# microsoft/timewarp

Measured on AMD Instinct MI355X. Metric: MH-accepted samples/sec (whole node), alanine-dipeptide kernel_transformer_nvp, higher is better.
Workload: dtype f16x3 (split-fp16 operands, 3 MFMAs per fp32 product, fp32 accumulate)

## Files before the change

### timewarp_amd/csrc/tw_api.hip

```cpp
#include "tw_common.h"

namespace tw {
std::atomic<int> g_debug_flags{0};
const char* last_error();
int launch_prior_logp(const float* zc, const float* zv, const uint8_t* masked, int64_t n_cond, const float* prior,
                      const float* delta, float sign, float* out, int64_t n_rows, int V, hipStream_t s);
int launch_uncentre_add(const float* xc, const float* com, const float* resid, int64_t n_cond, float* y, int V,
                        int displacement, int64_t n_rows, hipStream_t s);
int launch_sub(const float* a, const float* b, float* o, int64_t total, hipStream_t s);
int launch_kinetic(const float* v, const float* masses, int random_velocs, float kbT, float* out, int64_t n, int V,
                   hipStream_t s);
int launch_mh_accept(const float* energy, const float* p_xy, const float* p_yx, const float* u, const float* yc,
                     const float* yv, float* xc, float* xv, float* out_exp, float* out_pacc, uint8_t* out_acc,
                     int32_t* result, int64_t S, int V, hipStream_t s, int64_t n_chains = 1);
int launch_chirality(const float* coords, const int32_t* centres, const float* ref, int n_centres, uint8_t* changed,
                     int64_t n_rows, int V, hipStream_t s);
int amber_energy(const tw_forcefield* ff, const float* coords, double* out, double* terms, int64_t n, hipStream_t s);
int amber_energy_forces(const tw_forcefield* ff, const float* coords, double* out_energy, double* out_forces, int64_t n, hipStream_t s);
int langevin_steps(const tw_forcefield* ff, const float* masses, float* coords, float* velocs, int n_steps, double dt,
                   double friction, double kbT, int scheme, unsigned long long seed, long long step0, double* out_energy,
                   int64_t n, hipStream_t s);
}

using namespace tw;
// ... 135 lines not shown
  if (rc) return rc;
  TW_REQUIRE(h1_supported(*desc, 22), "single-MFMA path unsupported for this config");
  TW_REQUIRE(raw && packed_h1, "NULL buffer");
  return h3_pack_weights(*desc, raw, (char*)packed_h1, (hipStream_t)stream, true);
}

int64_t tw_flow_workspace_bytes(const tw_flow_desc* desc, int64_t n_rows, int32_t n_atoms) {
  if (check_desc(desc) || n_rows < 0 || n_atoms <= 0) return -1;
  const int64_t rows = n_rows > 0 ? n_rows : 1;
  int64_t a = simple_workspace_bytes(*desc, rows, n_atoms);
  int64_t b = fused_supported(*desc, n_atoms) ? fused_workspace_bytes(*desc, rows, n_atoms) : 0;
  if (h3_supported(*desc, n_atoms)) {
    const int64_t c = h3_workspace_bytes(*desc, rows, n_atoms);
    if (c > b) b = c;
  }
  const int64_t extra = 6 * ((rows * n_atoms * 3 * 4 + 255) / 256 * 256) + 4 * ((rows * 4 + 255) / 256 * 256);
  return (a > b ? a : b) + extra;
}

int tw_flow_pass(const tw_flow_desc* desc, const float* raw, const float* packed, const int32_t* atom_types,
                 const float* x_coords, const float* x_velocs, const uint8_t* masked, int64_t n_cond, float* z_coords,
                 float* z_velocs, float* delta_logp, int64_t n_rows, int32_t n_atoms, int32_t reverse, int32_t path,
                 void* workspace, int64_t workspace_bytes, void* stream) {
  int rc = check_desc(desc);
  if (rc) return rc;
  TW_REQUIRE(n_rows >= 0 && n_atoms > 0 && n_cond > 0, "bad sizes");
  TW_REQUIRE(n_rows % n_cond == 0, "n_rows (%lld) must be a multiple of n_cond (%lld)", (long long)n_rows,
             (long long)n_cond);
  if (n_rows == 0) return TW_OK;
  TW_REQUIRE(raw && atom_types && x_coords && x_velocs && masked && z_coords && z_velocs && delta_logp && workspace,
             "NULL pointer argument");
  int p;
  if ((rc = resolve_path(*desc, n_atoms, path, packed, &p))) return rc;
  FlowArgs a{desc, raw, packed, atom_types, x_coords, x_velocs, masked, n_cond, z_coords, z_velocs,
             delta_logp, n_rows, n_atoms, reverse, workspace, workspace_bytes, (hipStream_t)stream};
  if (p == TW_PATH_FUSED_H3 || p == TW_PATH_FUSED_H1) {
    a.h1 = p == TW_PATH_FUSED_H1 ? 1 : 0;
    return flow_pass_h3(a);
  }
  a.simple_h3 = p == TW_PATH_SIMPLE_H3 ? 1 : 0;
  return p == TW_PATH_FUSED ? flow_pass_fused(a) : flow_pass_simple(a);
}

static char* carve(char*& p, int64_t bytes) {
  char* r = p;
  p += (bytes + 255) / 256 * 256;
  return r;
}

int tw_flow_log_likelihood(const tw_flow_desc* desc, const float* raw, const float* packed, const int32_t* atom_types,
                           const float* x_coords, const float* x_velocs, const float* y_coords, const float* y_velocs,
                           const uint8_t* masked, float* out_logp, int64_t n_rows, int32_t n_atoms, int32_t path,
                           void* workspace, int64_t workspace_bytes, void* stream) {
  int rc = check_desc(desc);
  if (rc) return rc;
  TW_REQUIRE(n_rows >= 0 && n_atoms > 0, "bad sizes");
  if (n_rows == 0) return TW_OK;
  TW_REQUIRE(raw && atom_types && x_coords && x_velocs && y_coords && y_velocs && masked && out_logp && workspace,
             "NULL pointer argument");
  hipStream_t s = (hipStream_t)stream;
  const int64_t el = n_rows * n_atoms * 3;
  char* p = (char*)workspace;
  float* xc = (float*)carve(p, el * 4);
  float* zc = (float*)carve(p, el * 4);
  float* zv = (float*)carve(p, el * 4);
// ... 300 lines not shown
```

### timewarp_amd/csrc/tw_common.h

```cpp
#pragma once
#include <hip/hip_runtime.h>
#include <stdint.h>
#include <stdio.h>
#include <string.h>

#include <atomic>
#include <vector>

#include "../../include/timewarp_hip.h"

namespace tw {

void set_error(const char* fmt, ...);

#define TW_HIP_CHECK(expr)                                                              \
  do {                                                                                  \
    hipError_t _e = (expr);                                                             \
    if (_e != hipSuccess) {                                                             \
      tw::set_error("%s failed: %s (%s:%d)", #expr, hipGetErrorString(_e), __FILE__, __LINE__); \
      return TW_ERR_HIP;                                                                \
    }                                                                                   \
  } while (0)

#define TW_LAUNCH_CHECK() TW_HIP_CHECK(hipGetLastError())
// ... 72 lines not shown
struct PackedLayout {
  int64_t tiles_per_net;
  int64_t side_per_net;
  int64_t net_stride;
  int64_t total;
};
PackedLayout packed_layout(const tw_flow_desc& d);

struct FusedGeom {
  int nt;
  int mpw;
  int tile_mask;
};
bool fused_geom(int n_atoms, FusedGeom* g);
bool fused_geom_nt(int n_atoms, int nt, FusedGeom* g);

int launch_scores(const float* x, const uint8_t* masked, const float* ls, int H, int64_t B, int V,
                  int normalise, int use_mm, float* out, hipStream_t s, const float* coeffs = nullptr, int order = 0,
                  int force_zero = 0, _Float16* s_hi = nullptr, _Float16* s_lo = nullptr);
bool scores_split_direct(int V);
int launch_centre(const float* x, const uint8_t* masked, float* xc, float* com, int64_t n, int V,
                  hipStream_t s);

struct FlowArgs {
  const tw_flow_desc* desc;
  const float* raw;
  const float* packed;
  const int32_t* atom_types;
  const float* x_coords;
  const float* x_velocs;
  const uint8_t* masked;
  int64_t n_cond;
  float* z_coords;
  float* z_velocs;
  float* delta_logp;
  int64_t n_rows;
  int n_atoms;
  int reverse;
  void* ws;
  int64_t ws_bytes;
  hipStream_t stream;
  int h1 = 0;
  int simple_h3 = 0;
};
__device__ __forceinline__ float tw_cdist_mm(float qx, float qy, float qz, float mx, float my, float mz) {
#pragma clang fp contract(off)
  const float qn = (qx * qx + qy * qy) + qz * qz;
  const float mn = (mx * mx + my * my) + mz * mz;
  float acc = (-2.f * qx) * mx;
  acc = __builtin_fmaf(-2.f * qy, my, acc);
  acc = __builtin_fmaf(-2.f * qz, mz, acc);
  acc = acc + qn;
  acc = acc + mn;
  return sqrtf(fmaxf(acc, 0.f));
}

__device__ __forceinline__ float basis_value(float sc, const float* __restrict__ coeff, int order, float coeff_mean) {
  if (order <= 0) return expf(-(sc * sc));
  {
#pragma clang fp contract(off)
  const float x = sc * sc;
  const float rf = (x - 1.0f) / (x + 1.0f);
  const float rf2 = 2.0f * rf;
  float rprev = 1.0f, rcur = rf;
  float acc = (coeff[0] - coeff_mean) * rprev;
  if (order >= 2) acc = __builtin_fmaf(coeff[1] - coeff_mean, rcur, acc);
// ... 30 lines not shown
bool equivariant_desc_ok(const tw_flow_desc& d);
void equivariant_raw_layout(const tw_flow_desc& d, RawLayout* L);
int64_t equivariant_workspace_bytes(const tw_flow_desc& d, int64_t n_rows, int n_atoms);
int flow_pass_equivariant(const FlowArgs& a);
int debug_module_equivariant(const FlowArgs& a, int c, int net, const float* z_other, float* dump);
int flow_pass_fused(const FlowArgs& a);
int64_t simple_workspace_bytes(const tw_flow_desc& d, int64_t n_rows, int n_atoms);
int64_t fused_workspace_bytes(const tw_flow_desc& d, int64_t n_rows, int n_atoms);
int launch_coupling(const float* s_raw, const float* t, const uint8_t* masked, int64_t n_cond,
                    float* z_out, float* delta_logp, int64_t n_rows, int V, int reverse, hipStream_t s,
                    const float* z_in = nullptr, int* flag = nullptr);
int* nonfinite_flag_device_ptr();
inline int* flow_range_flag(const tw_flow_desc& d) { return d.range_flag ? d.range_flag : nonfinite_flag_device_ptr(); }

struct PrevCoupling {
  const float* s_raw;
  const float* t;
  const float* z_in;
  float* z_out;
  float* delta_logp;
  int* nonfinite;
  int reverse;
};
enum PackFormat { PACK_F32, PACK_PAIR, PACK_HI };
enum PackKind { PACK_TILES, PACK_FOLD, PACK_COPY, PACK_SCALAR };
struct PackGroup {
  const float* src;
  const float* wo;
  int64_t n;
};
struct PackOp {
  int kind, fmt, group;
  const float* src;
  const float* wo;
  int ld, rows_valid, cols_valid;
  int H, h;
  int row0, col0, n_ot, n_ks;
  int64_t n, n_pad;
  void* dst;
};
struct PackPlan {
  std::vector<PackGroup> groups;
  std::vector<PackOp> ops;
  int add_group(PackGroup g) { groups.push_back(g); return (int)groups.size() - 1; }
  int matrix_scale(const float* src, int64_t n) { return add_group({src, nullptr, n}); }
  int fold_scale(const float* wv, const float* wo, int H) { return add_group({wv, wo, H}); }
// ... 62 lines not shown
```

### timewarp_amd/csrc/tw_mh_step.hip

```cpp
#include "tw_common.h"

extern "C" int tw_flow_pass(const tw_flow_desc* desc, const float* raw, const float* packed, const int32_t* atom_types,
                            const float* x_coords, const float* x_velocs, const uint8_t* masked, int64_t n_cond,
                            float* z_coords, float* z_velocs, float* delta_logp, int64_t n_rows, int32_t n_atoms,
                            int32_t reverse, int32_t path, void* workspace, int64_t workspace_bytes, void* stream);
extern "C" int64_t tw_flow_workspace_bytes(const tw_flow_desc* desc, int64_t n_rows, int32_t n_atoms);

namespace tw {
int amber_energy(const tw_forcefield* ff, const float* coords, double* out, double* terms, int64_t n, hipStream_t s);

namespace {

__device__ __forceinline__ float wsum(float v) {
#pragma unroll
  for (int o = 32; o > 0; o >>= 1) v += __shfl_xor(v, o);
  return v;
}

__device__ __forceinline__ float row_prior(const float* zc, const float* zv, const uint8_t* mk, const float* prior, int V) {
  const float sc = expf(prior[0]), sv = expf(prior[1]);
  const float var_c = sc * sc, var_v = sv * sv;
  const float lsc = logf(sc), lsv = logf(sv);
  const float half_log_2pi = 0.91893853320467274178f;
  float ac = 0.f, av = 0.f;
  for (int i = threadIdx.x; i < 3 * V; i += 64) {
    const float keep = mk[i / 3] ? 0.f : 1.f;
    const float a = zc[i], b = zv[i];
    ac += keep * (-(a * a) / (2.f * var_c) - lsc - half_log_2pi);
// ... 37 lines not shown
  if (n < S) {
    for (int a = threadIdx.x; a < V; a += 64) {
      types_rep[n * V + a] = types[a];
      masked_rep[n * V + a] = masked[a];
    }
    const float p = row_prior(zc + n * 3 * V, zv + n * 3 * V, masked, prior, V);
    if (threadIdx.x == 0) {
      prior0[n] = p;
      delta[n] = 0.f;
    }
    return;
  }
  float com[3];
  row_com(x_coords, masked, V, com);
  for (int i = threadIdx.x; i < 3 * V; i += 64) {
    xc[i] = x_coords[i] - com[i % 3];
    zc[S * 3 * V + i] = x_coords[i];
  }
  if (threadIdx.x < 3) com_out[threadIdx.x] = com[threadIdx.x];
  const float ek = row_kinetic(x_velocs, masses, random_velocs, kbT, V);
  if (threadIdx.x == 0) ekin_x[0] = ek;
}

__global__ void mh_finish_kernel(float* __restrict__ zc , const float* __restrict__ yv,
                                 const float* __restrict__ x_coords, const float* __restrict__ x_velocs,
                                 const float* __restrict__ xc, const float* __restrict__ com,
                                 const uint8_t* __restrict__ masked, const float* __restrict__ masses,
                                 const float* __restrict__ prior0, float* __restrict__ delta, float* __restrict__ p_xy,
                                 float* __restrict__ ekin_y, uint8_t* __restrict__ chir, const int32_t* __restrict__ centres,
                                 const float* __restrict__ ref_signs, int n_centres, float* __restrict__ t_c,
                                 float* __restrict__ t_v, float* __restrict__ c_v, float* __restrict__ c_c,
                                 int displacement, int random_velocs, float kbT, int V) {
  extern __shared__ float ys[];
  const int64_t n = blockIdx.x;
  const float sgn = random_velocs ? 1.f : -1.f;
  float* zrow = zc + n * 3 * V;
  for (int i = threadIdx.x; i < 3 * V; i += 64) {
    const float base = xc[i] + com[i % 3];
    const float y = displacement ? base + zrow[i] : zrow[i];
    zrow[i] = y;
    ys[i] = y;
    t_c[n * 3 * V + i] = displacement ? x_coords[i] - y : x_coords[i];
    t_v[n * 3 * V + i] = sgn * x_velocs[i];
    c_v[n * 3 * V + i] = sgn * yv[n * 3 * V + i];
  }
  __syncthreads();
  float cy[3];
  row_com(ys, masked, V, cy);
  for (int i = threadIdx.x; i < 3 * V; i += 64) c_c[n * 3 * V + i] = ys[i] - cy[i % 3];
  const float ek = row_kinetic(yv + n * 3 * V, masses, random_velocs, kbT, V);
  if (threadIdx.x == 0) {
    p_xy[n] = prior0[n] + delta[n];
    delta[n] = 0.f;
    ekin_y[n] = ek;
    bool ch = false;
    for (int c = 0; c < n_centres; ++c) {
      const int i0 = centres[4 * c], i1 = centres[4 * c + 1], i2 = centres[4 * c + 2], i3 = centres[4 * c + 3];
      float a[3], b[3], d[3];
      for (int k = 0; k < 3; ++k) {
        a[k] = ys[3 * i1 + k] - ys[3 * i0 + k];
        b[k] = ys[3 * i2 + k] - ys[3 * i0 + k];
        d[k] = ys[3 * i3 + k] - ys[3 * i0 + k];
      }
      const float cx = b[1] * d[2] - b[2] * d[1];
      const float cyy = b[2] * d[0] - b[0] * d[2];
      const float cz = b[0] * d[1] - b[1] * d[0];
      const float dot = a[0] * cx + a[1] * cyy + a[2] * cz;
      const float s = (dot > 0.f) ? 1.f : ((dot < 0.f) ? -1.f : 0.f);
      if (s != ref_signs[c]) ch = true;
    }
    chir[n] = ch ? 1 : 0;
  }
}

__global__ void mh_pyx_kernel(const float* __restrict__ zc, const float* __restrict__ zv, const uint8_t* __restrict__ masked,
                              const float* __restrict__ prior, const float* __restrict__ delta, float* __restrict__ p_yx, int V) {
  const int64_t n = blockIdx.x;
  const float p = row_prior(zc + n * 3 * V, zv + n * 3 * V, masked, prior, V);
  if (threadIdx.x == 0) p_yx[n] = p - delta[n];
}

__global__ void mh_accept_full_kernel(const double* __restrict__ e_pot, const float* __restrict__ ekin_y,
                                      const float* __restrict__ ekin_x, const uint8_t* __restrict__ chir,
                                      const float* __restrict__ p_xy, const float* __restrict__ p_yx,
                                      const float* __restrict__ u, const float* __restrict__ yc, const float* __restrict__ yv,
                                      const float* __restrict__ x_coords, const float* __restrict__ x_velocs,
                                      float* __restrict__ new_c, float* __restrict__ new_v, float* __restrict__ stats,
                                      uint8_t* __restrict__ out_acc, int32_t* __restrict__ result, float inv_kbT,
                                      int64_t S, int V) {
  __shared__ int first;
  if (threadIdx.x == 0) first = 0x7fffffff;
  __syncthreads();
  const float epx = (float)e_pot[S] * inv_kbT;
  const float ekx = ekin_x[0];
  int local = 0x7fffffff;
  for (int64_t s = threadIdx.x; s < S; s += blockDim.x) {
    float epy = (float)e_pot[s] * inv_kbT;
    if (chir[s]) epy = epy + 2000.f;
    const float eky = ekin_y[s];
    const float dkin = eky - ekx;
    const float dpot = epy - epx;
    const float energy = dpot + dkin;
// ... 141 lines not shown
    if (threadIdx.x == 0) {
      prior0[n] = p;
      delta[n] = 0.f;
    }
    return;
  }
  const int c = (int)(n - rows);
  const float* x = x_coords + (int64_t)c * 3 * V;
  float* v = cur_v + (int64_t)c * 3 * V;
  for (int i = threadIdx.x; i < 3 * V; i += 64)
    v[i] = (dr.on && dr.resample) ? draw_normal(dr, c, 2, (uint32_t)i) : x_velocs[(int64_t)c * 3 * V + i];
  __syncthreads();
  float com[3];
  row_com(x, masked + c * V, V, com);
  for (int i = threadIdx.x; i < 3 * V; i += 64) {
    xc[(int64_t)c * 3 * V + i] = x[i] - com[i % 3];
    zc[(rows + c) * 3 * V + i] = x[i];
  }
  if (threadIdx.x < 3) com_out[3 * c + threadIdx.x] = com[threadIdx.x];
  const float ek = row_kinetic(v, masses, random_velocs, kbT, V);
  if (threadIdx.x == 0) ekin_x[c] = ek;
}

__global__ void mhc_finish_kernel(float* __restrict__ zc, const float* __restrict__ yv, const float* __restrict__ x_coords,
                                  const float* __restrict__ x_velocs, const float* __restrict__ xc,
                                  const float* __restrict__ com, const uint8_t* __restrict__ masked,
                                  const float* __restrict__ masses, const float* __restrict__ prior0,
                                  float* __restrict__ delta, float* __restrict__ p_xy, float* __restrict__ ekin_y,
                                  uint8_t* __restrict__ chir, const int32_t* __restrict__ centres,
                                  const float* __restrict__ ref_signs, int n_centres, float* __restrict__ t_c,
                                  float* __restrict__ t_v, float* __restrict__ c_v, float* __restrict__ c_c,
                                  int displacement, int random_velocs, float kbT, int C, int V) {
  extern __shared__ float ys[];
  const int64_t n = blockIdx.x;
  const int c = (int)(n % C);
  const float sgn = random_velocs ? 1.f : -1.f;
  const float *xq = x_coords + (int64_t)c * 3 * V, *xw = x_velocs + (int64_t)c * 3 * V, *xcc = xc + (int64_t)c * 3 * V;
  const uint8_t* mk = masked + c * V;
  float* zrow = zc + n * 3 * V;
  for (int i = threadIdx.x; i < 3 * V; i += 64) {
    const float base = xcc[i] + com[3 * c + i % 3];
    const float y = displacement ? base + zrow[i] : zrow[i];
    zrow[i] = y;
    ys[i] = y;
    t_c[n * 3 * V + i] = displacement ? xq[i] - y : xq[i];
    t_v[n * 3 * V + i] = sgn * xw[i];
    c_v[n * 3 * V + i] = sgn * yv[n * 3 * V + i];
  }
  __syncthreads();
  float cy[3];
  row_com(ys, mk, V, cy);
  for (int i = threadIdx.x; i < 3 * V; i += 64) c_c[n * 3 * V + i] = ys[i] - cy[i % 3];
  const float ek = row_kinetic(yv + n * 3 * V, masses, random_velocs, kbT, V);
  if (threadIdx.x == 0) {
    p_xy[n] = prior0[n] + delta[n];
    delta[n] = 0.f;
    ekin_y[n] = ek;
    bool ch = false;
    for (int q = 0; q < n_centres; ++q) {
      const int i0 = centres[4 * q], i1 = centres[4 * q + 1], i2 = centres[4 * q + 2], i3 = centres[4 * q + 3];
      float a[3], b[3], d[3];
      for (int k = 0; k < 3; ++k) {
        a[k] = ys[3 * i1 + k] - ys[3 * i0 + k];
        b[k] = ys[3 * i2 + k] - ys[3 * i0 + k];
        d[k] = ys[3 * i3 + k] - ys[3 * i0 + k];
      }
      const float cx = b[1] * d[2] - b[2] * d[1];
      const float cyy = b[2] * d[0] - b[0] * d[2];
      const float cz = b[0] * d[1] - b[1] * d[0];
      const float dot = a[0] * cx + a[1] * cyy + a[2] * cz;
      const float sg = (dot > 0.f) ? 1.f : ((dot < 0.f) ? -1.f : 0.f);
      if (sg != ref_signs[q]) ch = true;
    }
    chir[n] = ch ? 1 : 0;
  }
}

__global__ void mhc_pyx_kernel(const float* __restrict__ zc, const float* __restrict__ zv, const uint8_t* __restrict__ masked,
                               const float* __restrict__ prior, const float* __restrict__ delta, float* __restrict__ p_yx,
                               int C, int V) {
  const int64_t n = blockIdx.x;
  const float p = row_prior(zc + n * 3 * V, zv + n * 3 * V, masked + (n % C) * V, prior, V);
  if (threadIdx.x == 0) p_yx[n] = p - delta[n];
}

__global__ void mhc_accept_kernel(const double* __restrict__ e_pot, const float* __restrict__ ekin_y,
                                  const float* __restrict__ ekin_x, const uint8_t* __restrict__ chir,
                                  const float* __restrict__ p_xy, const float* __restrict__ p_yx,
                                  const float* __restrict__ u, const float* __restrict__ yc, const float* __restrict__ yv,
                                  const float* __restrict__ x_coords, const float* __restrict__ cur_v,
                                  float* __restrict__ new_c, float* __restrict__ new_v, float* __restrict__ stats,
                                  uint8_t* __restrict__ out_acc, int32_t* __restrict__ result, float inv_kbT, int64_t S, int C,
                                  int V) {
  __shared__ int first;
  const int c = blockIdx.x;
  const int64_t rows = S * C;
  if (threadIdx.x == 0) first = 0x7fffffff;
  __syncthreads();
  const float epx = (float)e_pot[rows + c] * inv_kbT;
  const float ekx = ekin_x[c];
  int local = 0x7fffffff;
  for (int64_t s = threadIdx.x; s < S; s += blockDim.x) {
    const int64_t n = s * C + c;
    float epy = (float)e_pot[n] * inv_kbT;
    if (chir[n]) epy = epy + 2000.f;
    const float eky = ekin_y[n];
// ... 86 lines not shown
  w.xc = (float*)take(C * V * 3 * 4);
  w.com = (float*)take(C * 3 * 4);
  w.prior0 = (float*)take(rows * 4);
  w.delta = (float*)take(rows * 4);
  w.ekin_x = (float*)take(C * 4);
  w.ekin_y = (float*)take(rows * 4);
  w.p_xy = (float*)take(rows * 4);
  w.p_yx = (float*)take(rows * 4);
  w.e_pot = (double*)take((rows + C) * 8);
  w.chir = (uint8_t*)take(rows);
  w.masked_rep = (uint8_t*)take(rows * V);
  w.types_rep = (int32_t*)take(rows * V * 4);
  w.t_c = (float*)take(el);
  w.t_v = (float*)take(el);
  w.c_v = (float*)take(el);
  w.c_c = (float*)take(el);
  w.flow = p;
  w.flow_bytes = tw_flow_workspace_bytes(d, rows, V);
  p += (w.flow_bytes + 255) / 256 * 256;
  w.bytes = p - (char*)base;
  return w;
}

}
}

using namespace tw;

extern "C" {

int64_t tw_mh_iteration_workspace_bytes(const tw_flow_desc* desc, int64_t n_proposals, int32_t n_atoms) {
  if (!desc || n_proposals <= 0 || n_atoms <= 0) return -1;
  if (tw_flow_workspace_bytes(desc, n_proposals, n_atoms) < 0) return -1;
  return step_ws(desc, n_proposals, n_atoms, nullptr).bytes;
}

int tw_mh_iteration(const tw_flow_desc* desc, const float* raw, const void* packed, int32_t path, const tw_forcefield* ff,
                    const tw_mh_options* opt, const int32_t* atom_types, const uint8_t* masked, int32_t n_atoms,
                    const float* x_coords, const float* x_velocs, float* zy_coords, float* zy_velocs, const float* u,
                    float* new_coords, float* new_velocs, float* out_stats, uint8_t* out_accepted, int32_t* result,
                    int64_t n_proposals, void* workspace, int64_t workspace_bytes, void* stream) {
  TW_REQUIRE(desc && raw && ff && opt && atom_types && masked && x_coords && x_velocs && zy_coords && zy_velocs && u &&
                 new_coords && new_velocs && out_stats && out_accepted && result && workspace,
             "NULL pointer argument");
  TW_REQUIRE(n_proposals > 0 && n_proposals < (1LL << 30) && n_atoms > 0, "bad sizes");
  TW_REQUIRE(ff->n_atoms == n_atoms, "force field is for %d atoms, the molecule has %d", ff->n_atoms, n_atoms);
  TW_REQUIRE(opt->kbT > 0.f, "kbT must be positive");
  TW_REQUIRE(opt->random_velocs || opt->masses, "masses are needed unless random_velocs");
  TW_REQUIRE(opt->n_centres == 0 || (opt->centres && opt->reference_signs), "chirality guard needs centres and signs");
  TW_REQUIRE(!desc->ignore_cond_velocity, "ignore_conditional_velocity models take the op-by-op route");
  const int64_t S = n_proposals;
  const int V = n_atoms;
  hipStream_t s = (hipStream_t)stream;
  const StepWs w = step_ws(desc, S, V, workspace);
  if (w.flow_bytes < 0) return TW_ERR_INVALID;
  if (w.bytes > workspace_bytes) {
    set_error("workspace too small: need %lld bytes, have %lld", (long long)w.bytes, (long long)workspace_bytes);
    return TW_ERR_WORKSPACE;
  }
  const RawLayout L = raw_layout(*desc);
  const float* prior = raw + L.prior;
  const float* masses = opt->masses ? opt->masses : x_velocs;
  int rc;
  hipLaunchKernelGGL(mh_begin_kernel, dim3((unsigned)(S + 1)), dim3(64), 0, s, x_coords, x_velocs, masked, masses, prior,
                     zy_coords, zy_velocs, w.xc, w.com, w.prior0, w.delta, w.ekin_x, atom_types, w.types_rep, w.masked_rep,
                     opt->random_velocs, opt->kbT, S, V);
  TW_LAUNCH_CHECK();
  if ((rc = tw_flow_pass(desc, raw, (const float*)packed, atom_types, w.xc, x_velocs, masked, 1, zy_coords, zy_velocs, w.delta,
                         S, V, 1, path, w.flow, w.flow_bytes, stream)))
    return rc;
  hipLaunchKernelGGL(mh_finish_kernel, dim3((unsigned)S), dim3(64), (size_t)3 * V * sizeof(float), s, zy_coords, zy_velocs,
                     x_coords, x_velocs, w.xc, w.com, masked, masses, w.prior0, w.delta, w.p_xy, w.ekin_y, w.chir,
                     opt->centres, opt->reference_signs, opt->n_centres, w.t_c, w.t_v, w.c_v, w.c_c, desc->displacement,
                     opt->random_velocs, opt->kbT, V);
  TW_LAUNCH_CHECK();
  static thread_local hipStream_t sides[32] = {};
  static thread_local hipEvent_t evs[32][2] = {};
  int dev_id = 0;
  TW_HIP_CHECK(hipGetDevice(&dev_id));
  TW_REQUIRE(dev_id >= 0 && dev_id < 32, "device index %d out of range", dev_id);
  if (!sides[dev_id]) {
    TW_HIP_CHECK(hipStreamCreateWithFlags(&sides[dev_id], hipStreamNonBlocking));
    TW_HIP_CHECK(hipEventCreateWithFlags(&evs[dev_id][0], hipEventDisableTiming));
    TW_HIP_CHECK(hipEventCreateWithFlags(&evs[dev_id][1], hipEventDisableTiming));
  }
  hipStream_t side = sides[dev_id];
  hipEvent_t ev_y = evs[dev_id][0], ev_e = evs[dev_id][1];
  const int dbg = g_debug_flags;
  const bool inline_energy = (dbg & TW_DEBUG_ENERGY_SIDE_STREAM)   ? false
                             : (dbg & TW_DEBUG_ENERGY_MAIN_STREAM) ? true
                                                                   : 2 * S * (int64_t)V >= (int64_t)160 * 192;
  if (inline_energy) {
    if ((rc = amber_energy(ff, zy_coords, w.e_pot, nullptr, S + 1, s))) return rc;
  } else {
    TW_HIP_CHECK(hipEventRecord(ev_y, s));
    TW_HIP_CHECK(hipStreamWaitEvent(side, ev_y, 0));
    if ((rc = amber_energy(ff, zy_coords, w.e_pot, nullptr, S + 1, side))) return rc;
    TW_HIP_CHECK(hipEventRecord(ev_e, side));
  }
  if ((rc = tw_flow_pass(desc, raw, (const float*)packed, w.types_rep, w.c_c, w.c_v, w.masked_rep, S, w.t_c, w.t_v, w.delta, S,
                         V, 0, path, w.flow, w.flow_bytes, stream)))
    return rc;
  hipLaunchKernelGGL(mh_pyx_kernel, dim3((unsigned)S), dim3(64), 0, s, w.t_c, w.t_v, masked, prior, w.delta, w.p_yx, V);
  TW_LAUNCH_CHECK();
  if (!inline_energy) TW_HIP_CHECK(hipStreamWaitEvent(s, ev_e, 0));
  hipLaunchKernelGGL(mh_accept_full_kernel, dim3(1), dim3(1024), 0, s, w.e_pot, w.ekin_y, w.ekin_x, w.chir, w.p_xy, w.p_yx, u,
                     zy_coords, zy_velocs, x_coords, x_velocs, new_coords, new_velocs, out_stats, out_accepted, result,
                     1.0f / opt->kbT, S, V);
  TW_LAUNCH_CHECK();
  return TW_OK;
}

int64_t tw_mh_iteration_chains_workspace_bytes(const tw_flow_desc* desc, int64_t n_proposals, int64_t n_chains, int32_t n_atoms) {
  if (!desc || n_proposals <= 0 || n_chains <= 0 || n_atoms <= 0) return -1;
  if (tw_flow_workspace_bytes(desc, n_proposals * n_chains, n_atoms) < 0) return -1;
  return chains_ws(desc, n_proposals, n_chains, n_atoms, nullptr).bytes;
}

int tw_mh_iteration_chains(const tw_flow_desc* desc, const float* raw, const void* packed, int32_t path, const tw_forcefield* ff,
                           const tw_mh_options* opt, const tw_mh_draws* draws, const int32_t* atom_types, const uint8_t* masked,
                           int32_t n_atoms, const float* x_coords, const float* x_velocs, float* cur_velocs, float* zy_coords,
                           float* zy_velocs, float* u, float* new_coords, float* new_velocs, float* out_stats,
                           uint8_t* out_accepted, int32_t* result, int64_t n_proposals, int64_t n_chains, void* workspace,
                           int64_t workspace_bytes, void* stream) {
  TW_REQUIRE(desc && raw && ff && opt && atom_types && masked && x_coords && x_velocs && cur_velocs && zy_coords && zy_velocs &&
                 u && new_coords && new_velocs && out_stats && out_accepted && result && workspace,
             "NULL pointer argument");
  TW_REQUIRE(n_proposals > 0 && n_chains > 0 && n_atoms > 0 && n_proposals * n_chains < (1LL << 30), "bad sizes");
// ... 4 lines not shown
  TW_REQUIRE(opt->n_centres == 0 || (opt->centres && opt->reference_signs), "chirality guard needs centres and signs");
  TW_REQUIRE(!desc->ignore_cond_velocity, "ignore_conditional_velocity models take the op-by-op route");
  TW_REQUIRE(!draws || (draws->iteration >= 0 && draws->first_chain >= 0), "draws: negative iteration or chain id");
  TW_REQUIRE(!draws || !draws->resample_velocs || opt->random_velocs, "draws: resampled velocities need random_velocs");
  TW_REQUIRE(!draws || n_proposals * 3 * (int64_t)n_atoms < (1LL << 32), "draws: a chain's latent stream has 2^32 elements");
  const int64_t S = n_proposals, rows = n_proposals * n_chains;
  const int Cn = (int)n_chains, V = n_atoms;
  hipStream_t s = (hipStream_t)stream;
  const ChainsWs w = chains_ws(desc, S, n_chains, V, workspace);
  if (w.flow_bytes < 0) return TW_ERR_INVALID;
  if (w.bytes > workspace_bytes) {
    set_error("workspace too small: need %lld bytes, have %lld", (long long)w.bytes, (long long)workspace_bytes);
    return TW_ERR_WORKSPACE;
  }
  const RawLayout L = raw_layout(*desc);
  const float* prior = raw + L.prior;
  const float* masses = opt->masses ? opt->masses : x_velocs;
  const Draws dr = make_draws(draws);
  int rc;
  hipLaunchKernelGGL(mhc_begin_kernel, dim3((unsigned)(rows + Cn)), dim3(64), 0, s, x_coords, x_velocs, masked, masses, prior,
                     zy_coords, zy_velocs, u, cur_velocs, w.xc, w.com, w.prior0, w.delta, w.ekin_x, atom_types, w.types_rep,
                     w.masked_rep, opt->random_velocs, opt->kbT, S, Cn, V, dr);
  TW_LAUNCH_CHECK();
  if ((rc = tw_flow_pass(desc, raw, (const float*)packed, atom_types, w.xc, cur_velocs, masked, n_chains, zy_coords, zy_velocs,
                         w.delta, rows, V, 1, path, w.flow, w.flow_bytes, stream)))
    return rc;
  hipLaunchKernelGGL(mhc_finish_kernel, dim3((unsigned)rows), dim3(64), (size_t)3 * V * sizeof(float), s, zy_coords, zy_velocs,
                     x_coords, cur_velocs, w.xc, w.com, masked, masses, w.prior0, w.delta, w.p_xy, w.ekin_y, w.chir,
                     opt->centres, opt->reference_signs, opt->n_centres, w.t_c, w.t_v, w.c_v, w.c_c, desc->displacement,
                     opt->random_velocs, opt->kbT, Cn, V);
  TW_LAUNCH_CHECK();
  if ((rc = amber_energy(ff, zy_coords, w.e_pot, nullptr, rows + Cn, s))) return rc;
  if ((rc = tw_flow_pass(desc, raw, (const float*)packed, w.types_rep, w.c_c, w.c_v, w.masked_rep, rows, w.t_c, w.t_v, w.delta,
                         rows, V, 0, path, w.flow, w.flow_bytes, stream)))
    return rc;
  hipLaunchKernelGGL(mhc_pyx_kernel, dim3((unsigned)rows), dim3(64), 0, s, w.t_c, w.t_v, masked, prior, w.delta, w.p_yx, Cn, V);
  TW_LAUNCH_CHECK();
  hipLaunchKernelGGL(mhc_accept_kernel, dim3((unsigned)Cn), dim3(S >= 512 ? 1024 : 256), 0, s, w.e_pot, w.ekin_y, w.ekin_x,
                     w.chir, w.p_xy, w.p_yx, u, zy_coords, zy_velocs, x_coords, cur_velocs, new_coords, new_velocs, out_stats,
                     out_accepted, result, 1.0f / opt->kbT, S, Cn, V);
  TW_LAUNCH_CHECK();
  return TW_OK;
}

int tw_mh_draw_chains(const tw_flow_desc* desc, const float* raw, const tw_mh_draws* draws, float* z_coords, float* z_velocs,
                      float* u, float* velocs, int64_t n_proposals, int64_t n_chains, int32_t n_atoms, void* stream) {
  TW_REQUIRE(desc && raw && draws, "NULL pointer argument");
  TW_REQUIRE(n_proposals >= 0 && n_chains > 0 && n_atoms > 0 && n_proposals * n_chains < (1LL << 30), "bad sizes");
  TW_REQUIRE(draws->iteration >= 0 && draws->first_chain >= 0, "draws: negative iteration or chain id");
  TW_REQUIRE(n_proposals * 3 * (int64_t)n_atoms < (1LL << 32), "draws: a chain's latent stream has 2^32 elements");
  const RawLayout L = raw_layout(*desc);
  hipLaunchKernelGGL(mhc_draws_kernel, dim3((unsigned)(n_proposals * n_chains + n_chains)), dim3(64), 0, (hipStream_t)stream,
                     raw + L.prior, z_coords, z_velocs, u, velocs, n_proposals, (int)n_chains, n_atoms, make_draws(draws));
  TW_LAUNCH_CHECK();
  return TW_OK;
}

}
```

### timewarp_amd/csrc/tw_netblock_h3.hip

```cpp
#include <utility>
#include <vector>

#include "tw_common.h"

namespace tw {

typedef float f4 __attribute__((ext_vector_type(4)));
typedef _Float16 h8 __attribute__((ext_vector_type(8)));
typedef _Float16 h4 __attribute__((ext_vector_type(4)));
typedef unsigned u4 __attribute__((ext_vector_type(4)));
typedef unsigned u2 __attribute__((ext_vector_type(2)));

#define H3_NT 3
#define H3_FFN_SPLIT 4
#define H3_TOK (16 * H3_NT)
#define H3_XT 48
#define H3_XT_IMG 1536
#define H3_PAIR_BYTES 2048
#define H3_STAGE_PAIRS 4
#define H3_STAGE_TILE_BYTES 8192
#define H3_STAGE_BYTES 9216
#define H3_RING 5
#define H3_XT_BYTES (128 * H3_XT * 2)
#define H3_WAVE_LDS (2 * H3_XT_BYTES)
// ... 2772 lines not shown
  if (g_debug_flags & TW_DEBUG_SEPARATE_COUPLING) {
    for (int i = 0; i < d.n_coupling; ++i) {
      const int c = a.reverse ? d.n_coupling - 1 - i : i;
      const bool positions = (c % 2) == d.pos_mod2;
      if (kernel_attention && d.cheb_order > 0 && (rc = h3_score_frags(a, L, fg, w, shared, c, &vb))) return rc;
      if ((rc = h3_launch(a, L, fg, c, -1, positions ? a.z_velocs : a.z_coords, w.sfrag, vb, shared, w.s_out, w.t_out, nullptr)))
        return rc;
      if ((rc = launch_coupling(w.s_out, w.t_out, a.masked, a.n_cond, positions ? a.z_coords : a.z_velocs, a.delta_logp,
                                a.n_rows, a.n_atoms, a.reverse, a.stream, nullptr, flag)))
        return rc;
    }
    return TW_OK;
  }
  for (int i = 0; i < d.n_coupling; ++i) {
    const int c = a.reverse ? d.n_coupling - 1 - i : i;
    const bool positions = (c % 2) == d.pos_mod2;
    tv = positions ? 0 : 1;
    const int ov = 1 - tv;
    if (prev.s_raw) {
      prev.z_in = cur[ov];
      prev.z_out = alt[ov];
    }
    if (kernel_attention && d.cheb_order > 0 && (rc = h3_score_frags(a, L, fg, w, shared, c, &vb))) return rc;
    if ((rc = h3_launch(a, L, fg, c, -1, cur[ov], w.sfrag, vb, shared, sbuf[i & 1], tbuf[i & 1], nullptr, prev))) return rc;
    if (prev.s_raw) std::swap(cur[ov], alt[ov]);
    prev = PrevCoupling{sbuf[i & 1], tbuf[i & 1], nullptr, nullptr, a.delta_logp, flag, a.reverse};
  }
  if ((rc = launch_coupling(prev.s_raw, prev.t, a.masked, a.n_cond, caller[tv], a.delta_logp, a.n_rows, a.n_atoms, a.reverse,
                            a.stream, cur[tv], flag)))
    return rc;
  const int ov = 1 - tv;
  if (cur[ov] != caller[ov])
    TW_HIP_CHECK(hipMemcpyAsync(caller[ov], cur[ov], (size_t)a.n_rows * a.n_atoms * 3 * sizeof(float), hipMemcpyDeviceToDevice,
                                a.stream));
  return TW_OK;
}

bool h3_ffn_tokens_supported(const tw_flow_desc& d) { return h3_supported(d, 22); }

int h3_ffn_tokens(const tw_flow_desc& d, const void* packed, int coupling, int net, int layer, float* h, int64_t n_tokens,
                  hipStream_t stream, float* scratch, int64_t scratch_floats, const void* split_stages) {
  TW_REQUIRE(packed && h3_ffn_tokens_supported(d), "FFN on the split-fp16 stream: unsupported model or no stream");
  const H3Geom g = h3_geom(d);
  const int64_t att_stages = d.variant == 1 ? 4LL * g.H : 8LL * g.H;
  const int64_t first = (int64_t)(g.in_a_stages + 2) * g.hid_chunks + (int64_t)layer * (att_stages + 4LL * g.ff_chunks) + att_stages;
  const char* net_base = (const char*)packed + (int64_t)(coupling * 2 + net) * g.net_stride_bytes;
  H3FfnParams p;
  p.stages = net_base + first * H3_STAGE_BYTES;
  p.side = (const float*)(net_base + g.stages * H3_STAGE_BYTES) + g.side_layers + (int64_t)layer * g.side_layer_size;
  p.h = h;
  p.n_tokens = n_tokens;
  p.ff_chunks = g.ff_chunks;
// ... 159 lines not shown
```

Baseline: 156.2.

## Fuse final coupling into MH finish/pyx kernels and overlap energy with score fragments

The flow pass gains a hook that defers the last affine coupling. The last coupling is then applied inside mh_finish/mh_pyx (and the chain variants) per row, instead of running as a separate launch_coupling kernel. On the fused h3 path the potential-energy evaluation is also forked onto a side stream, so it runs beside the first coupling's score-fragment work, and is joined before the first network launch. This removes one kernel launch plus a round trip through memory per pass and hides energy latency. The cost is extra event synchronisation and dropped __restrict__ qualifiers on the finish kernels.

```diff
diff --git a/timewarp_amd/csrc/tw_api.hip b/timewarp_amd/csrc/tw_api.hip
--- a/timewarp_amd/csrc/tw_api.hip
+++ b/timewarp_amd/csrc/tw_api.hip
@@ -181,6 +181,16 @@
                  const float* x_coords, const float* x_velocs, const uint8_t* masked, int64_t n_cond, float* z_coords,
                  float* z_velocs, float* delta_logp, int64_t n_rows, int32_t n_atoms, int32_t reverse, int32_t path,
                  void* workspace, int64_t workspace_bytes, void* stream) {
+  return tw::flow_pass_hooked(desc, raw, packed, atom_types, x_coords, x_velocs, masked, n_cond, z_coords, z_velocs, delta_logp,
+                              n_rows, n_atoms, reverse, path, workspace, workspace_bytes, stream, nullptr);
+}
+
+}
+
+int tw::flow_pass_hooked(const tw_flow_desc* desc, const float* raw, const float* packed, const int32_t* atom_types,
+                         const float* x_coords, const float* x_velocs, const uint8_t* masked, int64_t n_cond, float* z_coords,
+                         float* z_velocs, float* delta_logp, int64_t n_rows, int32_t n_atoms, int32_t reverse, int32_t path,
+                         void* workspace, int64_t workspace_bytes, void* stream, FlowHooks* hooks) {
   int rc = check_desc(desc);
   if (rc) return rc;
   TW_REQUIRE(n_rows >= 0 && n_atoms > 0 && n_cond > 0, "bad sizes");
@@ -195,11 +205,14 @@
              delta_logp, n_rows, n_atoms, reverse, workspace, workspace_bytes, (hipStream_t)stream};
   if (p == TW_PATH_FUSED_H3 || p == TW_PATH_FUSED_H1) {
     a.h1 = p == TW_PATH_FUSED_H1 ? 1 : 0;
+    a.hooks = hooks;
     return flow_pass_h3(a);
   }
   a.simple_h3 = p == TW_PATH_SIMPLE_H3 ? 1 : 0;
   return p == TW_PATH_FUSED ? flow_pass_fused(a) : flow_pass_simple(a);
 }
+
+extern "C" {
 
 static char* carve(char*& p, int64_t bytes) {
   char* r = p;
diff --git a/timewarp_amd/csrc/tw_common.h b/timewarp_amd/csrc/tw_common.h
--- a/timewarp_amd/csrc/tw_common.h
+++ b/timewarp_amd/csrc/tw_common.h
@@ -118,6 +118,7 @@
 int launch_centre(const float* x, const uint8_t* masked, float* xc, float* com, int64_t n, int V,
                   hipStream_t s);
 
+struct FlowHooks;
 struct FlowArgs {
   const tw_flow_desc* desc;
   const float* raw;
@@ -138,6 +139,7 @@
   hipStream_t stream;
   int h1 = 0;
   int simple_h3 = 0;
+  FlowHooks* hooks = nullptr;
 };
 __device__ __forceinline__ float tw_cdist_mm(float qx, float qy, float qz, float mx, float my, float mz) {
 #pragma clang fp contract(off)
@@ -214,6 +216,35 @@
   int* nonfinite;
   int reverse;
 };
+struct FlowHooks {
+  hipEvent_t join = nullptr;
+  bool joined = false;
+  PrevCoupling last{};
+};
+int flow_pass_hooked(const tw_flow_desc* desc, const float* raw, const float* packed, const int32_t* atom_types,
+                     const float* x_coords, const float* x_velocs, const uint8_t* masked, int64_t n_cond, float* z_coords,
+                     float* z_velocs, float* delta_logp, int64_t n_rows, int32_t n_atoms, int32_t reverse, int32_t path,
+                     void* workspace, int64_t workspace_bytes, void* stream, FlowHooks* hooks);
+#ifdef __HIPCC__
+__device__ __forceinline__ float row_coupling(const PrevCoupling& pc, const uint8_t* __restrict__ mask_row, int64_t n, int V, int lane) {
+  float acc = 0.f;
+  bool bad = false;
+  for (int i = lane; i < 3 * V; i += 64) {
+    const int64_t idx = n * 3 * V + i;
+    const float scale = expf(pc.s_raw[idx]);
+    const float shift = pc.t[idx];
+    bad |= !(isfinite(pc.s_raw[idx]) && isfinite(shift));
+    const float keep = mask_row[i / 3] ? 0.f : 1.f;
+    acc += logf(scale) * keep;
+    pc.z_out[idx] = pc.reverse ? (pc.z_in[idx] - shift) / scale : pc.z_in[idx] * scale + shift;
+  }
+  if (bad) atomicOr(pc.nonfinite, 1);
+#pragma unroll
+  for (int o = 32; o > 0; o >>= 1) acc += __shfl_xor(acc, o);
+  const float logdet = pc.reverse ? -acc : acc;
+  return pc.delta_logp[n] - logdet;
+}
+#endif
 enum PackFormat { PACK_F32, PACK_PAIR, PACK_HI };
 enum PackKind { PACK_TILES, PACK_FOLD, PACK_COPY, PACK_SCALAR };
 struct PackGroup {
diff --git a/timewarp_amd/csrc/tw_mh_step.hip b/timewarp_amd/csrc/tw_mh_step.hip
--- a/timewarp_amd/csrc/tw_mh_step.hip
+++ b/timewarp_amd/csrc/tw_mh_step.hip
@@ -1,9 +1,5 @@
 #include "tw_common.h"
 
-extern "C" int tw_flow_pass(const tw_flow_desc* desc, const float* raw, const float* packed, const int32_t* atom_types,
-                            const float* x_coords, const float* x_velocs, const uint8_t* masked, int64_t n_cond,
-                            float* z_coords, float* z_velocs, float* delta_logp, int64_t n_rows, int32_t n_atoms,
-                            int32_t reverse, int32_t path, void* workspace, int64_t workspace_bytes, void* stream);
 extern "C" int64_t tw_flow_workspace_bytes(const tw_flow_desc* desc, int64_t n_rows, int32_t n_atoms);
 
 namespace tw {
@@ -87,18 +83,25 @@
   if (threadIdx.x == 0) ekin_x[0] = ek;
 }
 
-__global__ void mh_finish_kernel(float* __restrict__ zc , const float* __restrict__ yv,
+__global__ void mh_finish_kernel(float* zc , const float* yv,
                                  const float* __restrict__ x_coords, const float* __restrict__ x_velocs,
                                  const float* __restrict__ xc, const float* __restrict__ com,
                                  const uint8_t* __restrict__ masked, const float* __restrict__ masses,
-                                 const float* __restrict__ prior0, float* __restrict__ delta, float* __restrict__ p_xy,
+                                 const float* __restrict__ prior0, float* delta, float* __restrict__ p_xy,
                                  float* __restrict__ ekin_y, uint8_t* __restrict__ chir, const int32_t* __restrict__ centres,
                                  const float* __restrict__ ref_signs, int n_centres, float* __restrict__ t_c,
                                  float* __restrict__ t_v, float* __restrict__ c_v, float* __restrict__ c_c,
-                                 int displacement, int random_velocs, float kbT, int V) {
+                                 int displacement, int random_velocs, float kbT, int V, PrevCoupling last) {
   extern __shared__ float ys[];
   const int64_t n = blockIdx.x;
   const float sgn = random_velocs ? 1.f : -1.f;
+  float dl;
+  if (last.s_raw) {
+    dl = row_coupling(last, masked, n, V, threadIdx.x);
+    __syncthreads();
+  } else {
+    dl = delta[n];
+  }
   float* zrow = zc + n * 3 * V;
   for (int i = threadIdx.x; i < 3 * V; i += 64) {
     const float base = xc[i] + com[i % 3];
@@ -115,7 +118,7 @@
   for (int i = threadIdx.x; i < 3 * V; i += 64) c_c[n * 3 * V + i] = ys[i] - cy[i % 3];
   const float ek = row_kinetic(yv + n * 3 * V, masses, random_velocs, kbT, V);
   if (threadIdx.x == 0) {
-    p_xy[n] = prior0[n] + delta[n];
+    p_xy[n] = prior0[n] + dl;
     delta[n] = 0.f;
     ekin_y[n] = ek;
     bool ch = false;
@@ -138,11 +141,19 @@
   }
 }
 
-__global__ void mh_pyx_kernel(const float* __restrict__ zc, const float* __restrict__ zv, const uint8_t* __restrict__ masked,
-                              const float* __restrict__ prior, const float* __restrict__ delta, float* __restrict__ p_yx, int V) {
+__global__ void mh_pyx_kernel(const float* zc, const float* zv, const uint8_t* __restrict__ masked,
+                              const float* __restrict__ prior, const float* delta, float* __restrict__ p_yx, int V,
+                              PrevCoupling last) {
   const int64_t n = blockIdx.x;
+  float dl;
+  if (last.s_raw) {
+    dl = row_coupling(last, masked, n, V, threadIdx.x);
+    __syncthreads();
+  } else {
+    dl = delta[n];
+  }
   const float p = row_prior(zc + n * 3 * V, zv + n * 3 * V, masked, prior, V);
-  if (threadIdx.x == 0) p_yx[n] = p - delta[n];
+  if (threadIdx.x == 0) p_yx[n] = p - dl;
 }
 
 __global__ void mh_accept_full_kernel(const double* __restrict__ e_pot, const float* __restrict__ ekin_y,
@@ -330,21 +341,28 @@
   if (threadIdx.x == 0) ekin_x[c] = ek;
 }
 
-__global__ void mhc_finish_kernel(float* __restrict__ zc, const float* __restrict__ yv, const float* __restrict__ x_coords,
+__global__ void mhc_finish_kernel(float* zc, const float* yv, const float* __restrict__ x_coords,
                                   const float* __restrict__ x_velocs, const float* __restrict__ xc,
                                   const float* __restrict__ com, const uint8_t* __restrict__ masked,
                                   const float* __restrict__ masses, const float* __restrict__ prior0,
-                                  float* __restrict__ delta, float* __restrict__ p_xy, float* __restrict__ ekin_y,
+                                  float* delta, float* __restrict__ p_xy, float* __restrict__ ekin_y,
                                   uint8_t* __restrict__ chir, const int32_t* __restrict__ centres,
                                   const float* __restrict__ ref_signs, int n_centres, float* __restrict__ t_c,
                                   float* __restrict__ t_v, float* __restrict__ c_v, float* __restrict__ c_c,
-                                  int displacement, int random_velocs, float kbT, int C, int V) {
+                                  int displacement, int random_velocs, float kbT, int C, int V, PrevCoupling last) {
   extern __shared__ float ys[];
   const int64_t n = blockIdx.x;
   const int c = (int)(n % C);
   const float sgn = random_velocs ? 1.f : -1.f;
   const float *xq = x_coords + (int64_t)c * 3 * V, *xw = x_velocs + (int64_t)c * 3 * V, *xcc = xc + (int64_t)c * 3 * V;
   const uint8_t* mk = masked + c * V;
+  float dl;
+  if (last.s_raw) {
+    dl = row_coupling(last, mk, n, V, threadIdx.x);
+    __syncthreads();
+  } else {
+    dl = delta[n];
+  }
   float* zrow = zc + n * 3 * V;
   for (int i = threadIdx.x; i < 3 * V; i += 64) {
     const float base = xcc[i] + com[3 * c + i % 3];
@@ -361,7 +379,7 @@
   for (int i = threadIdx.x; i < 3 * V; i += 64) c_c[n * 3 * V + i] = ys[i] - cy[i % 3];
   const float ek = row_kinetic(yv + n * 3 * V, masses, random_velocs, kbT, V);
   if (threadIdx.x == 0) {
-    p_xy[n] = prior0[n] + delta[n];
+    p_xy[n] = prior0[n] + dl;
     delta[n] = 0.f;
     ekin_y[n] = ek;
     bool ch = false;
@@ -384,12 +402,20 @@
   }
 }
 
-__global__ void mhc_pyx_kernel(const float* __restrict__ zc, const float* __restrict__ zv, const uint8_t* __restrict__ masked,
-                               const float* __restrict__ prior, const float* __restrict__ delta, float* __restrict__ p_yx,
-                               int C, int V) {
+__global__ void mhc_pyx_kernel(const float* zc, const float* zv, const uint8_t* __restrict__ masked,
+                               const float* __restrict__ prior, const float* delta, float* __restrict__ p_yx, int C, int V,
+                               PrevCoupling last) {
   const int64_t n = blockIdx.x;
-  const float p = row_prior(zc + n * 3 * V, zv + n * 3 * V, masked + (n % C) * V, prior, V);
-  if (threadIdx.x == 0) p_yx[n] = p - delta[n];
+  const uint8_t* mk = masked + (n % C) * V;
+  float dl;
+  if (last.s_raw) {
+    dl = row_coupling(last, mk, n, V, threadIdx.x);
+    __syncthreads();
+  } else {
+    dl = delta[n];
+  }
+  const float p = row_prior(zc + n * 3 * V, zv + n * 3 * V, mk, prior, V);
+  if (threadIdx.x == 0) p_yx[n] = p - dl;
 }
 
 __global__ void mhc_accept_kernel(const double* __restrict__ e_pot, const float* __restrict__ ekin_y,
@@ -522,6 +548,54 @@
   return w;
 }
 
+int mh_side_stream(hipStream_t* side, hipEvent_t* ev_fork, hipEvent_t* ev_join) {
+  static thread_local hipStream_t sides[32] = {};
+  static thread_local hipEvent_t evs[32][2] = {};
+  int dev_id = 0;
+  TW_HIP_CHECK(hipGetDevice(&dev_id));
+  TW_REQUIRE(dev_id >= 0 && dev_id < 32, "device index %d out of range", dev_id);
+  if (!sides[dev_id]) {
+    TW_HIP_CHECK(hipStreamCreateWithFlags(&sides[dev_id], hipStreamNonBlocking));
+    TW_HIP_CHECK(hipEventCreateWithFlags(&evs[dev_id][0], hipEventDisableTiming));
+    TW_HIP_CHECK(hipEventCreateWithFlags(&evs[dev_id][1], hipEventDisableTiming));
+  }
+  *side = sides[dev_id];
+  *ev_fork = evs[dev_id][0];
+  *ev_join = evs[dev_id][1];
+  return TW_OK;
+}
+
+bool energy_beside_fragments(const tw_flow_desc* d, int path) {
+  return (path == TW_PATH_FUSED_H3 || path == TW_PATH_FUSED_H1) && d->variant == 0 && !(g_debug_flags & TW_DEBUG_ENERGY_MAIN_STREAM);
+}
+
+int fork_energy(const tw_forcefield* ff, const float* coords, double* out, int64_t n, hipStream_t s, FlowHooks* hooks) {
+  hipStream_t side;
+  hipEvent_t ev_fork, ev_join;
+  int rc;
+  if ((rc = mh_side_stream(&side, &ev_fork, &ev_join))) return rc;
+  TW_HIP_CHECK(hipEventRecord(ev_fork, s));
+  TW_HIP_CHECK(hipStreamWaitEvent(side, ev_fork, 0));
+  rc = amber_energy(ff, coords, out, nullptr, n, side);
+  const hipError_t e1 = hipEventRecord(ev_join, side);
+  if (rc || e1 != hipSuccess) {
+    (void)hipStreamSynchronize(side);
+    if (rc) return rc;
+    TW_HIP_CHECK(e1);
+  }
+  hooks->join = ev_join;
+  hooks->joined = false;
+  return TW_OK;
+}
+
+int join_energy(hipStream_t s, FlowHooks* hooks) {
+  if (hooks->join && !hooks->joined) {
+    hooks->joined = true;
+    TW_HIP_CHECK(hipStreamWaitEvent(s, hooks->join, 0));
+  }
+  return TW_OK;
+}
+
 }
 }
 
@@ -566,44 +640,45 @@
                      zy_coords, zy_velocs, w.xc, w.com, w.prior0, w.delta, w.ekin_x, atom_types, w.types_rep, w.masked_rep,
                      opt->random_velocs, opt->kbT, S, V);
   TW_LAUNCH_CHECK();
-  if ((rc = tw_flow_pass(desc, raw, (const float*)packed, atom_types, w.xc, x_velocs, masked, 1, zy_coords, zy_velocs, w.delta,
-                         S, V, 1, path, w.flow, w.flow_bytes, stream)))
+  FlowHooks rev;
+  if ((rc = flow_pass_hooked(desc, raw, (const float*)packed, atom_types, w.xc, x_velocs, masked, 1, zy_coords, zy_velocs, w.delta,
+                             S, V, 1, path, w.flow, w.flow_bytes, stream, &rev)))
     return rc;
   hipLaunchKernelGGL(mh_finish_kernel, dim3((unsigned)S), dim3(64), (size_t)3 * V * sizeof(float), s, zy_coords, zy_velocs,
                      x_coords, x_velocs, w.xc, w.com, masked, masses, w.prior0, w.delta, w.p_xy, w.ekin_y, w.chir,
                      opt->centres, opt->reference_signs, opt->n_centres, w.t_c, w.t_v, w.c_v, w.c_c, desc->displacement,
-                     opt->random_velocs, opt->kbT, V);
-  TW_LAUNCH_CHECK();
-  static thread_local hipStream_t sides[32] = {};
-  static thread_local hipEvent_t evs[32][2] = {};
-  int dev_id = 0;
-  TW_HIP_CHECK(hipGetDevice(&dev_id));
-  TW_REQUIRE(dev_id >= 0 && dev_id < 32, "device index %d out of range", dev_id);
-  if (!sides[dev_id]) {
-    TW_HIP_CHECK(hipStreamCreateWithFlags(&sides[dev_id], hipStreamNonBlocking));
-    TW_HIP_CHECK(hipEventCreateWithFlags(&evs[dev_id][0], hipEventDisableTiming));
-    TW_HIP_CHECK(hipEventCreateWithFlags(&evs[dev_id][1], hipEventDisableTiming));
-  }
-  hipStream_t side = sides[dev_id];
-  hipEvent_t ev_y = evs[dev_id][0], ev_e = evs[dev_id][1];
+                     opt->random_velocs, opt->kbT, V, rev.last);
+  TW_LAUNCH_CHECK();
+  hipStream_t side;
+  hipEvent_t ev_y, ev_e;
+  if ((rc = mh_side_stream(&side, &ev_y, &ev_e))) return rc;
   const int dbg = g_debug_flags;
   const bool inline_energy = (dbg & TW_DEBUG_ENERGY_SIDE_STREAM)   ? false
                              : (dbg & TW_DEBUG_ENERGY_MAIN_STREAM) ? true
                                                                    : 2 * S * (int64_t)V >= (int64_t)160 * 192;
-  if (inline_energy) {
+  FlowHooks fwd;
+  if (inline_energy && energy_beside_fragments(desc, path)) {
+    if ((rc = fork_energy(ff, zy_coords, w.e_pot, S + 1, s, &fwd))) return rc;
+  } else if (inline_energy) {
     if ((rc = amber_energy(ff, zy_coords, w.e_pot, nullptr, S + 1, s))) return rc;
   } else {
     TW_HIP_CHECK(hipEventRecord(ev_y, s));
     TW_HIP_CHECK(hipStreamWaitEvent(side, ev_y, 0));
-    if ((rc = amber_energy(ff, zy_coords, w.e_pot, nullptr, S + 1, side))) return rc;
-    TW_HIP_CHECK(hipEventRecord(ev_e, side));
-  }
-  if ((rc = tw_flow_pass(desc, raw, (const float*)packed, w.types_rep, w.c_c, w.c_v, w.masked_rep, S, w.t_c, w.t_v, w.delta, S,
-                         V, 0, path, w.flow, w.flow_bytes, stream)))
-    return rc;
-  hipLaunchKernelGGL(mh_pyx_kernel, dim3((unsigned)S), dim3(64), 0, s, w.t_c, w.t_v, masked, prior, w.delta, w.p_yx, V);
-  TW_LAUNCH_CHECK();
+    rc = amber_energy(ff, zy_coords, w.e_pot, nullptr, S + 1, side);
+    const hipError_t e1 = hipEventRecord(ev_e, side);
+    if (rc || e1 != hipSuccess) {
+      (void)hipStreamSynchronize(side);
+      if (rc) return rc;
+      TW_HIP_CHECK(e1);
+    }
+  }
+  rc = flow_pass_hooked(desc, raw, (const float*)packed, w.types_rep, w.c_c, w.c_v, w.masked_rep, S, w.t_c, w.t_v, w.delta, S, V, 0,
+                        path, w.flow, w.flow_bytes, stream, &fwd);
   if (!inline_energy) TW_HIP_CHECK(hipStreamWaitEvent(s, ev_e, 0));
+  const int jrc = join_energy(s, &fwd);
+  if (rc || jrc) return rc ? rc : jrc;
+  hipLaunchKernelGGL(mh_pyx_kernel, dim3((unsigned)S), dim3(64), 0, s, w.t_c, w.t_v, masked, prior, w.delta, w.p_yx, V, fwd.last);
+  TW_LAUNCH_CHECK();
   hipLaunchKernelGGL(mh_accept_full_kernel, dim3(1), dim3(1024), 0, s, w.e_pot, w.ekin_y, w.ekin_x, w.chir, w.p_xy, w.p_yx, u,
                      zy_coords, zy_velocs, x_coords, x_velocs, new_coords, new_velocs, out_stats, out_accepted, result,
                      1.0f / opt->kbT, S, V);
@@ -654,19 +729,27 @@
                      zy_coords, zy_velocs, u, cur_velocs, w.xc, w.com, w.prior0, w.delta, w.ekin_x, atom_types, w.types_rep,
                      w.masked_rep, opt->random_velocs, opt->kbT, S, Cn, V, dr);
   TW_LAUNCH_CHECK();
-  if ((rc = tw_flow_pass(desc, raw, (const float*)packed, atom_types, w.xc, cur_velocs, masked, n_chains, zy_coords, zy_velocs,
-                         w.delta, rows, V, 1, path, w.flow, w.flow_bytes, stream)))
+  FlowHooks rev;
+  if ((rc = flow_pass_hooked(desc, raw, (const float*)packed, atom_types, w.xc, cur_velocs, masked, n_chains, zy_coords, zy_velocs,
+                             w.delta, rows, V, 1, path, w.flow, w.flow_bytes, stream, &rev)))
     return rc;
   hipLaunchKernelGGL(mhc_finish_kernel, dim3((unsigned)rows), dim3(64), (size_t)3 * V * sizeof(float), s, zy_coords, zy_velocs,
                      x_coords, cur_velocs, w.xc, w.com, masked, masses, w.prior0, w.delta, w.p_xy, w.ekin_y, w.chir,
                      opt->centres, opt->reference_signs, opt->n_centres, w.t_c, w.t_v, w.c_v, w.c_c, desc->displacement,
-                     opt->random_velocs, opt->kbT, Cn, V);
-  TW_LAUNCH_CHECK();
-  if ((rc = amber_energy(ff, zy_coords, w.e_pot, nullptr, rows + Cn, s))) return rc;
-  if ((rc = tw_flow_pass(desc, raw, (const float*)packed, w.types_rep, w.c_c, w.c_v, w.masked_rep, rows, w.t_c, w.t_v, w.delta,
-                         rows, V, 0, path, w.flow, w.flow_bytes, stream)))
+                     opt->random_velocs, opt->kbT, Cn, V, rev.last);
+  TW_LAUNCH_CHECK();
+  FlowHooks fwd;
+  if (energy_beside_fragments(desc, path)) {
+    if ((rc = fork_energy(ff, zy_coords, w.e_pot, rows + Cn, s, &fwd))) return rc;
+  } else if ((rc = amber_energy(ff, zy_coords, w.e_pot, nullptr, rows + Cn, s))) {
     return rc;
-  hipLaunchKernelGGL(mhc_pyx_kernel, dim3((unsigned)rows), dim3(64), 0, s, w.t_c, w.t_v, masked, prior, w.delta, w.p_yx, Cn, V);
+  }
+  rc = flow_pass_hooked(desc, raw, (const float*)packed, w.types_rep, w.c_c, w.c_v, w.masked_rep, rows, w.t_c, w.t_v, w.delta, rows,
+                        V, 0, path, w.flow, w.flow_bytes, stream, &fwd);
+  const int jrc = join_energy(s, &fwd);
+  if (rc || jrc) return rc ? rc : jrc;
+  hipLaunchKernelGGL(mhc_pyx_kernel, dim3((unsigned)rows), dim3(64), 0, s, w.t_c, w.t_v, masked, prior, w.delta, w.p_yx, Cn, V,
+                     fwd.last);
   TW_LAUNCH_CHECK();
   hipLaunchKernelGGL(mhc_accept_kernel, dim3((unsigned)Cn), dim3(S >= 512 ? 1024 : 256), 0, s, w.e_pot, w.ekin_y, w.ekin_x,
                      w.chir, w.p_xy, w.p_yx, u, zy_coords, zy_velocs, x_coords, cur_velocs, new_coords, new_velocs, out_stats,
diff --git a/timewarp_amd/csrc/tw_netblock_h3.hip b/timewarp_amd/csrc/tw_netblock_h3.hip
--- a/timewarp_amd/csrc/tw_netblock_h3.hip
+++ b/timewarp_amd/csrc/tw_netblock_h3.hip
@@ -2818,12 +2818,20 @@
       prev.z_out = alt[ov];
     }
     if (kernel_attention && d.cheb_order > 0 && (rc = h3_score_frags(a, L, fg, w, shared, c, &vb))) return rc;
+    if (i == 0 && a.hooks && a.hooks->join) {
+      TW_HIP_CHECK(hipStreamWaitEvent(a.stream, a.hooks->join, 0));
+      a.hooks->joined = true;
+    }
     if ((rc = h3_launch(a, L, fg, c, -1, cur[ov], w.sfrag, vb, shared, sbuf[i & 1], tbuf[i & 1], nullptr, prev))) return rc;
     if (prev.s_raw) std::swap(cur[ov], alt[ov]);
     prev = PrevCoupling{sbuf[i & 1], tbuf[i & 1], nullptr, nullptr, a.delta_logp, flag, a.reverse};
   }
-  if ((rc = launch_coupling(prev.s_raw, prev.t, a.masked, a.n_cond, caller[tv], a.delta_logp, a.n_rows, a.n_atoms, a.reverse,
-                            a.stream, cur[tv], flag)))
+  if (a.hooks && prev.s_raw) {
+    prev.z_in = cur[tv];
+    prev.z_out = caller[tv];
+    a.hooks->last = prev;
+  } else if ((rc = launch_coupling(prev.s_raw, prev.t, a.masked, a.n_cond, caller[tv], a.delta_logp, a.n_rows, a.n_atoms, a.reverse,
+                                   a.stream, cur[tv], flag)))
     return rc;
   const int ov = 1 - tv;
   if (cur[ov] != caller[ov])
```

After: 155.2. No clear change (-0.7%).
